# JaworWr/CUDA-ray-tracer

Measured on AMD Instinct MI355X. Metric: Mrays/sec, 20spheres.yml @1920x1080, higher is better.
Workload: dtype f64

## Files before the change

cuda-ray-tracer_amd/csrc/rt_capi.cpp:

```cpp
#include <hip/hip_runtime.h>

#include <algorithm>
#include <cmath>
#include <cstdarg>
#include <cstdio>
#include <cstdlib>
#include <cstring>
#include <memory>
#include <new>
#include <string>
#include <vector>

#include "mi355rt.h"
#include "rt_launch.h"
#include "rt_scene_dev.h"
#include "rt_scene_image.hpp"
#include "rt_frame_host.hpp"
#include "rt_set_scene.h"
#include "scene-exception.h"
#include "scene.h"
#include "camera.h"

#define RT_KERNELS(V)                                                                                                                              \
    {RT_CAT(rt_launch_trace, V), RT_CAT(rt_launch_wavefront, V),  RT_CAT(rt_launch_ray_list, V),      RT_CAT(rt_launch_gbuffer, V),   RT_CAT(rt_launch_pick, V), \
// ... 161 lines not shown
    DevMem<void> d_fb;
    DevMem<unsigned long long> d_counters;
    Event ev0, ev1;
    Event ev_done;

    hipStream_t last_stream = nullptr;
    bool rendered = false;
    bool captured = false;
    bool counted = false;
    bool zero_counters = false;
    DevMem<uint64_t> d_stamps;
    DevMem<double> d_camx, d_camy;
    size_t n_stamp_rows = 0;
    uint64_t frame = 0;
    uint32_t tag = 0;
    DevMem<uint32_t> d_order, d_tiles;
    MappedWords h_listed;
    uint32_t ord_split = 0;
    std::vector<double> cub_coefs;
    bool lean_ok = false;
    bool lean_now = true;
    uint32_t wg_slots = 1536;
    int lean_force = 0;
    bool ord_on = true;
    Staging pick;
    Staging ext;
    Staging rq;
    Scratch pth;
    DevMem<SetSceneStatus> d_ss_status;
    DevMem<unsigned char> d_ss_stage;
};

#ifdef RT_DIAGNOSTIC_BUILD
extern "C" int rt_abi_version(void) { return RT_ABI_VERSION | RT_ABI_DIAGNOSTIC; }
#else
extern "C" int rt_abi_version(void) { return RT_ABI_VERSION; }
#endif

extern "C" const char *rt_last_error(void) { return g_last_error.c_str(); }

extern "C" void rt_set_last_error(const char *message) { g_last_error = message ? message : ""; }

template <typename F>
static int scene_handle(rt_scene **out, F &&make)
{
    std::unique_ptr<rt_scene> s(new rt_scene());
// ... 207 lines not shown
    std::memset(&fa, 0, sizeof(fa));
    fa.aspect = (double) rw / rh;
    fa.tan_half_fov = std::tan(0.5 * sd->vertical_fov);
    fa.bg[0] = sd->bg_color[0];
    fa.bg[1] = sd->bg_color[1];
    fa.bg[2] = sd->bg_color[2];
    fa.bg[3] = 1.0f;
    fa.width = rw;
    fa.height = rh;
    fa.max_refl = sd->max_reflections;
    fa.rank = cfg.rank;
    fa.world = cfg.world;
    fa.band_rows = kf * cfg.band_rows;
    fa.local_rows = kf * ctx->local_rows;
    fa.tiles_x = (rw + RT_TILE - 1) / RT_TILE;
    fa.n_tiles = fa.tiles_x * ((fa.local_rows + RT_TILE - 1) / RT_TILE);
    fa.rgba8 = (ctx->ssaa == 1u && cfg.format == RT_FMT_RGBA8) ? 1u : 0u;
    fa.ord_plain = (cfg.flags & RT_FLAG_PLAIN_ORDER) ? 1u : 0u;
    ctx->ord_split = (cfg.flags & RT_FLAG_NOSPLIT) ? 0u : RT_ORD_SPLIT_CLASSES;
    if (const char *e = std::getenv("MI355RT_SPLIT_CLASSES")) ctx->ord_split = (uint32_t) std::atoi(e) & 15u;
    int cus = 0;
    if (hipDeviceGetAttribute(&cus, hipDeviceAttributeMultiprocessorCount, device) == hipSuccess && cus > 0) ctx->wg_slots = 6u * (uint32_t) cus;
    if (const char *e = std::getenv("MI355RT_LEAN")) ctx->lean_force = (e[0] == 'a') ? 1 : ((e[0] == 'n') ? -1 : 0);
}

static int create_scene(rt_ctx *ctx, const rt_scene_desc *sd, rtp::SceneImage &im)
{
    FrameArgs &fa = ctx->fa;
    im = rtp::scene_image(*sd, ctx->cfg.flags, fa);
    ctx->cub_coefs = im.cub_coefs;
    ctx->lean_ok = im.lean_ok && !std::getenv("MI355RT_NOLEAN");
    if (!(ctx->cfg.flags & RT_FLAG_SIMPLE)) {
        const size_t lds = rt_wavefront_lds_bytes_strict(fa.stage_bytes, sd->n_lights, (int) fa.has_mirror, fa.cull ? fa.n_us : 0u, 0, fa.n_cub);
        if (lds > 160u * 1024u) return fail(RT_ERR_SCENE, "rt_create: scene needs %zu bytes of LDS per workgroup (limit 160 KiB)", lds);
    }
    if (ctx->adaptive && (size_t) sd->n_objects * (sizeof(DevObject) + sizeof(UsEntry)) > 160u * 1024u)
        return fail(RT_ERR_SCENE, "rt_create: adaptive supersampling stages %zu bytes of LDS per workgroup (limit 160 KiB)",
                    (size_t) sd->n_objects * (sizeof(DevObject) + sizeof(UsEntry)));
    if (ctx->geometry && rt_gbuffer_lds_bytes_strict(&fa) > 160u * 1024u)
        return fail(RT_ERR_SCENE, "rt_create: RT_FLAG_SSAA_GEOMETRY stages %zu bytes of LDS per workgroup (limit 160 KiB)", rt_gbuffer_lds_bytes_strict(&fa));
    return RT_OK;
}

static int create_device_state(rt_ctx *ctx, const rtp::SceneImage &im)
{
    const FrameArgs &fa = ctx->fa;
// ... 44 lines not shown
    if (!ctx->geometry) return RT_OK;
    const size_t hpx = (size_t) ctx->halo_slots * width;
    std::vector<uint32_t> xy(2u * hpx);
    for (uint32_t h = 0; h < ctx->halo_slots; h++) {
        const int64_t gy = rtf::halo_global_row(h, cfg.band_rows, cfg.world, cfg.rank, ctx->local_rows);
        const uint32_t row = (uint32_t) std::min<int64_t>(std::max<int64_t>(gy, 0), (int64_t) height - 1);
        for (uint32_t x = 0; x < width; x++) {
            xy[2u * ((size_t) h * width + x)] = x;
            xy[2u * ((size_t) h * width + x) + 1u] = row;
        }
    }
    RT_TRY("hipMalloc(object plane)", ctx->d_geo_obj.alloc((px ? px : 1u) * sizeof(int32_t)));
    RT_TRY("hipMalloc(normal plane)", ctx->d_geo_nrm.alloc((px ? px : 1u) * 16u));
    if (!hpx) return RT_OK;
    RT_TRY("hipMalloc(halo records)", ctx->d_geo_halo.alloc(sizeof(rt_hit) * hpx));
    return device_table(ctx->d_geo_xy, xy.data(), sizeof(uint32_t) * 2u * hpx, "halo coordinates");
}

static int create_order_state(rt_ctx *ctx)
{
    FrameArgs &fa = ctx->fa;
    const uint32_t flags = ctx->cfg.flags;
    if (!(flags & (RT_FLAG_SIMPLE | RT_FLAG_STATIC_ORDER)) && fa.n_tiles > 0 && fa.n_tiles <= RT_ORD_MAX_TILES) {
        fa.ord_stride = (RT_ORD_HDR + 17u * fa.n_tiles + 15u) & ~15u;
        if (int rc = device_table(ctx->d_order, nullptr, sizeof(uint32_t) * (3u * (size_t) fa.ord_stride + fa.n_tiles), "order")) return rc;
        fa.order_state = ctx->d_order;
        if (hipHostMalloc((void **) &ctx->h_listed.p, 64, hipHostMallocMapped | hipHostMallocPortable) == hipSuccess) {
            ctx->h_listed[0] = 0;
            ctx->h_listed[1] = 0;
            ctx->h_listed[2] = 0xFFFFFFFFu;
            if (hipHostGetDevicePointer((void **) &fa.ord_host, ctx->h_listed, 0) != hipSuccess) {
                ctx->h_listed.reset();
                fa.ord_host = nullptr;
            }
        } else {
            ctx->h_listed.p = nullptr;
            (void) hipGetLastError();
        }
    }
    if (!(flags & RT_FLAG_SIMPLE) && fa.all_cullable && fa.n_tiles > 0) {
        if (int rc = device_table(ctx->d_tiles, nullptr, sizeof(uint32_t) * fa.n_tiles, "tile state")) return rc;
        fa.tile_state = ctx->d_tiles;
    }
    ctx->zero_counters = std::getenv("MI355RT_DEBUG_COUNTERS") != nullptr;
    if (ctx->zero_counters) {
        ctx->n_stamp_rows = (size_t) fa.n_tiles * 9 + 96;
        if (ctx->d_stamps.alloc(ctx->n_stamp_rows * 16 * sizeof(uint64_t) + 8) != hipSuccess) ctx->d_stamps.p = nullptr;
// ... 93 lines not shown
static int timer_begin(rt_ctx *ctx, hipStream_t stream, const float *ms)
{
    if (ms) RT_HIP(hipEventRecord(ctx->ev0, stream));
    return RT_OK;
}

static int timer_end(rt_ctx *ctx, hipStream_t stream, float *ms)
{
    if (!ms) return RT_OK;
    RT_HIP(hipEventRecord(ctx->ev1, stream));
    RT_HIP(hipEventSynchronize(ctx->ev1));
    RT_HIP(hipEventElapsedTime(ms, ctx->ev0, ctx->ev1));
    return RT_OK;
}

static void choose_schedule(rt_ctx *ctx, FrameArgs &fa)
{
    if (ctx->lean_ok && ctx->h_listed && ctx->lean_force == 0) {
        const uint32_t tiles = ((volatile uint32_t *) ctx->h_listed.p)[2];
        if (ctx->lean_now ? (uint64_t) tiles * 100u < (uint64_t) ctx->wg_slots * 62u : (uint64_t) tiles * 100u >= (uint64_t) ctx->wg_slots * 66u) ctx->lean_now = !ctx->lean_now;
    } else {
        ctx->lean_now = ctx->lean_force >= 0;
    }
    static const bool debug_order = std::getenv("MI355RT_DEBUG_ORDER") != nullptr;
    if (debug_order && ctx->h_listed)
        std::fprintf(stderr, "mi355rt: frame %llu: tiles with hits %u, list slots wanted %u, census %u, schedule %s\n", (unsigned long long) ctx->frame, ((volatile uint32_t *) ctx->h_listed.p)[2],
                     ((volatile uint32_t *) ctx->h_listed.p)[0], ((volatile uint32_t *) ctx->h_listed.p)[1], ctx->lean_now ? "lean" : "general");
    fa.lean = (ctx->lean_ok && ctx->lean_now && !fa.sparse) ? 1u : 0u;
}

static int rotate_launch_order(rt_ctx *ctx, FrameArgs &fa, hipStream_t stream)
{
    fa.ord_read = (uint32_t) (ctx->frame % 3u);
    fa.ord_write = (uint32_t) ((ctx->frame + 1u) % 3u);
    fa.ord_zero = (uint32_t) ((ctx->frame + 2u) % 3u);
    uint32_t cap = fa.n_tiles;
    if (ctx->h_listed) {
        const uint32_t seen = ((volatile uint32_t *) ctx->h_listed.p)[0], census = ((volatile uint32_t *) ctx->h_listed.p)[1];
        const uint64_t want = (uint64_t) seen + seen / 4u + 64u;
        if (want < cap) cap = (uint32_t) want;
        const uint64_t with_hits = (uint64_t) census * 16u;
        const uint64_t slots = ctx->wg_slots ? ctx->wg_slots : 1536u;
        const bool too_many = ctx->ord_on ? with_hits * 3u >= slots * 16u : with_hits >= slots * 4u;
        const bool too_dense = ctx->ord_on ? with_hits * 4u >= fa.n_tiles : with_hits * 5u >= fa.n_tiles;
        ctx->ord_on = !(too_many || too_dense);
    }
    fa.ord_cap = cap;
    fa.ord_on = ctx->ord_on ? 1u : 0u;
    fa.ord_split = (fa.sparse || fa.lean) ? 0u : ctx->ord_split;
    fa.ord_frame = (uint32_t) (ctx->frame % 0xFFFFFFF0ull) + 1u;
    if (fa.ord_frame == 1u && ctx->frame != 0u)
        RT_HIP(hipMemsetAsync(fa.order_state + 3u * (size_t) fa.ord_stride, 0, sizeof(uint32_t) * fa.n_tiles, stream));
    ctx->frame++;
    return RT_OK;
}

static int render_impl(rt_ctx *ctx, const double cam[16], void *dev_fb, void *stream_, float *ms, bool sparse, uint32_t sparse_cap)
{
    hipStream_t stream = (hipStream_t) stream_;
    FrameArgs &fa = ctx->fa;
    const bool ss = ctx->ssaa > 1u && !ctx->adaptive;
    const bool kernel_sparse = sparse && ctx->ssaa == 1u;
    fa.sparse = kernel_sparse ? 1u : 0u;
    fa.sparse_cap = kernel_sparse ? sparse_cap : 0u;
    choose_schedule(ctx, fa);
    rtf::frame_camera(fa, cam, ctx->cub_coefs);
    if (int rc = use_device(ctx)) return rc;
    bool capturing = false;
    if (int rc = order_begin("rt_render", ctx, stream, &capturing)) return rc;
    void *out = dev_fb ? dev_fb : ctx->d_fb.p;
    void *fb = ss ? ctx->d_ss.p : out;
// ... 721 lines not shown
```

cuda-ray-tracer_amd/csrc/rt_scene_dev.h:

```cpp
#ifndef RT_SCENE_DEV_H
#define RT_SCENE_DEV_H

#include <stddef.h>
#include <stdint.h>

enum {
    K_X3 = 0, K_Y3, K_Z3, K_X2Y, K_XY2, K_X2Z, K_XZ2, K_Y2Z, K_YZ2, K_XYZ,
    K_X2, K_Y2, K_Z2, K_XY, K_XZ, K_YZ,
    K_X, K_Y, K_Z, K_C
};

#define RT_CLS_CUBIC 1u
#define RT_CLS_SQUARE 2u
#define RT_CLS_CROSS 4u
#define RT_CLS_UNITSQ 8u

struct alignas(16) DevObject {
    double c[20];
    float albedo[3];
    float refl;
    uint32_t cls;
    uint32_t pad[3];
    double bs_center[3];
    double bs_radius;
// ... 69 lines not shown
    uint32_t has_mirror;
    uint32_t all_cullable;
    double tile_nt[9];
    double cx_a, cx_b;
    double cy_a, cy_b;
    uint32_t tile_planes_ok;
    uint32_t sparse, sparse_cap;
    uint32_t *order_state;
    uint32_t *ord_host;
    uint32_t ord_stride, ord_read, ord_write, ord_zero;
    uint32_t ord_cap;
    uint32_t ord_on;
    uint32_t ord_plain;
    uint32_t ord_frame;
    uint32_t ord_split;
    uint32_t *tile_state;
    uint32_t frame_tag;
    uint32_t n_scan;
    uint32_t lean;
    double cub_rec[4][10];
    double cub_abs[4][4];
    uint32_t lights_plain;
    uint32_t pt_mask[2];
};

#define RT_CUB_AT_MAX 4
#define RT_CUB_REC 10
static_assert(offsetof(FrameArgs, cub_abs) == offsetof(FrameArgs, cub_rec) + sizeof(double) * 4 * RT_CUB_REC, "cub_abs directly behind cub_rec");
#define RT_TILE 16
#define RT_SCAN_TILES 64
#define RT_PAINT_TILES 16
#define RT_ORD_SPLIT_CLASSES 8u
#define RT_ORD_HDR 32
#define RT_ORD_MAX_TILES 262144u

#endif
```

cuda-ray-tracer_amd/csrc/rt_wavefront.hip:

```cpp
#include <hip/hip_runtime.h>
#include <cstdlib>

#include "rt_launch.h"
#include "rt_math.hpp"
#include "rt_scene_dev.h"
#include "rt_wavefront_math.hpp"

#ifndef RT_VARIANT
#error "define RT_VARIANT=strict|fast"
#endif

namespace RT_SYM(rtw) {

using namespace rtm;

#define RT_LOAD_LIGHTK(lk, l) \
    LightK lk; \
    lk.p[0] = clight[l].p[0]; lk.p[1] = clight[l].p[1]; lk.p[2] = clight[l].p[2]; \
    lk.sdir[0] = clight[l].sdir[0]; lk.sdir[1] = clight[l].sdir[1]; lk.sdir[2] = clight[l].sdir[2]; \
    lk.u2 = clight[l].u2; lk.inv_uu = clight[l].inv_uu; lk.len_u = clight[l].len_u; lk.four_u2 = clight[l].four_u2; \
    lk.s_yz = clight[l].s_yz; lk.s_xz = clight[l].s_xz; lk.s_xy = clight[l].s_xy; \
    lk.color[0] = clight[l].color[0]; lk.color[1] = clight[l].color[1]; lk.color[2] = clight[l].color[2]; \
    lk.flags = clight[l].flags;
typedef const __attribute__((address_space(4))) LightK *ConstLights;
// ... 239 lines not shown
#pragma unroll
    for (uint32_t c = 0; c + 1 < ORD_CLASSES; c++) {
        const bool next = (k == c) && idx >= h.cnt[c];
        idx -= next ? h.cnt[c] : 0u;
        k += next ? 1u : 0u;
    }
}
__device__ __forceinline__ uint32_t ord_first(const OrdHeader &h, uint32_t k)
{
    uint32_t f = 0;
#pragma unroll
    for (uint32_t c = 0; c + 1 < ORD_CLASSES; c++) f += c < k ? h.cnt[c] : 0u;
    return f;
}
__device__ __forceinline__ uint32_t ord_rank_of_slot(uint32_t q, uint32_t n_eff, uint32_t first_block)
{
    const uint32_t off = first_block & 255u, row = (q + off) >> 8;
    if (!(row & 1u)) return q;
    const uint32_t lo = row * 256u - off;
    const uint32_t hi = (row + 1u) * 256u - off < n_eff ? (row + 1u) * 256u - off : n_eff;
    return lo + (hi - 1u - q);
}

constexpr uint32_t ST_EMPTY = 1u, ST_NONEMPTY = 2u, ST_TIMEOUT = 3u, ST_COVERED = 4u;
constexpr uint32_t ST_BITS = 3u, ST_MASK = 7u;
#ifndef RT_TILE_MAX_POLLS
#define RT_TILE_MAX_POLLS 48
#endif

__device__ __forceinline__ uint32_t tile_word_load(uint32_t *w) { return __hip_atomic_load(w, __ATOMIC_RELAXED, __HIP_MEMORY_SCOPE_AGENT); }

__device__ __forceinline__ uint32_t tile_word_wait(uint32_t *w, uint32_t tag, uint32_t v)
{
    for (int it = 0; (v >> ST_BITS) != tag; ++it) {
        if (it >= RT_TILE_MAX_POLLS) {
            uint32_t expect = v;
            if (__hip_atomic_compare_exchange_strong(w, &expect, (tag << ST_BITS) | ST_TIMEOUT, __ATOMIC_RELAXED, __ATOMIC_RELAXED, __HIP_MEMORY_SCOPE_AGENT))
                v = (tag << ST_BITS) | ST_TIMEOUT;
            else
                v = expect;
        } else {
            __builtin_amdgcn_s_sleep(16);
            v = tile_word_load(w);
        }
    }
    return v;
}

template <bool COUNT>
__device__ __forceinline__ void classify_tiles(const FrameArgs &fa, const UsEntry *us, uint32_t n_us, uint32_t *tile_state, uint32_t tag, uint32_t n_tiles,
                                               const uint32_t *ord_rd, uint32_t ord_cap, uint32_t ord_split, uint32_t wave, uint32_t lane, Cnt<COUNT> &cnt)
{
    const uint32_t i = lane & 15u, sl = lane >> 4;
    const uint32_t t = blockIdx.x * RT_SCAN_TILES + wave * 16u + i;
    const bool tv = t < n_tiles;
    uint32_t old = 0;
    if (sl == 0 && tv) old = tile_word_load(tile_state + t);
    double kx = 0.0, ky = 0.0, kz = 0.0, r = 0.0, inv = 0.0;
    if (sl < n_us) {
        const UsEntry *e = us + sl;
        kx = e->kx; ky = e->ky; kz = e->kz; r = e->r; inv = e->inv_r;
    }
    const uint32_t tc = tv ? t : n_tiles - 1u;
    const uint32_t tile_x = tc % fa.tiles_x, tile_y = tc / fa.tiles_x;
    const uint32_t x0 = tile_x * RT_TILE, y0l = tile_y * RT_TILE;
    const uint32_t x1 = x0 + RT_TILE - 1 < fa.width ? x0 + RT_TILE - 1 : fa.width - 1;
    const uint32_t y1l = y0l + RT_TILE - 1 < fa.local_rows ? y0l + RT_TILE - 1 : fa.local_rows - 1;
    const double gy0 = (double) global_row(fa, y0l), gy1 = (double) global_row(fa, y1l);
    const TilePlanes P = tile_planes(fa, fa.cx_a * ((double) x0 - 0.5) + fa.cx_b, fa.cx_a * ((double) x1 + 0.5) + fa.cx_b,
                                     fa.cy_a * (gy0 - 0.5) + fa.cy_b, fa.cy_a * (gy1 + 0.5) + fa.cy_b);
    const D3 org{fa.origin[0], fa.origin[1], fa.origin[2]};
    bool rel = sl < n_us && sphere_in_pyramid(kx, ky, kz, r, inv, org, P);
    for (uint32_t base = 4; base < n_us; base += 4) {
        const uint32_t j = base + sl;
        if (j < n_us) {
            const UsEntry *e = us + j;
            rel = rel || sphere_in_pyramid(e->kx, e->ky, e->kz, e->r, e->inv_r, org, P);
        }
    }
    if (!fa.tile_planes_ok) rel = true;
    unsigned long long m = __ballot(rel);
    m |= m >> 32;
    m |= m >> 16;
    const bool nonempty = (m >> i) & 1ull;
    if (sl == 0 && tv && (old >> ST_BITS) != tag) {
        uint32_t st = nonempty ? ST_NONEMPTY : ST_EMPTY;
        if (nonempty && ord_rd) {
            const OrdHeader oh = ord_header(ord_rd, ord_split);
            const uint32_t n_eff = ord_positions(oh) < ord_cap ? ord_positions(oh) : ord_cap;
            const uint32_t w = ord_rd[RT_ORD_HDR + t];
            const uint32_t cls = w & 31u, pos = w >> 5;
            if (cls >= 1u && cls <= ORD_CLASSES && pos < n_tiles) {
                const uint32_t k = cls - 1u;
                uint32_t count = 0;
#pragma unroll
                for (uint32_t c = 0; c < ORD_CLASSES; c++) count = c == k ? oh.cnt[c] : count;
                if (pos < count && ord_last_position(oh, ord_first(oh, k) + pos) < n_eff && ord_rd[RT_ORD_HDR + (1u + k) * n_tiles + pos] == t) st = ST_COVERED;
            }
        }
        uint32_t expect = old;
        __hip_atomic_compare_exchange_strong(tile_state + t, &expect, (tag << ST_BITS) | st, __ATOMIC_RELAXED, __ATOMIC_RELAXED,
                                             __HIP_MEMORY_SCOPE_AGENT);
    }
    if (lane == 0) {
        const uint32_t first = blockIdx.x * RT_SCAN_TILES + wave * 16u;
        const uint32_t nt = first >= n_tiles ? 0u : (n_tiles - first < 16u ? n_tiles - first : 16u);
        cnt.cull(C_TILE, (unsigned long long) nt * n_us);
    }
}

// ... 575 lines not shown
                if (hit) {
                    res.x = (acc.x < 1.0f) ? acc.x : 1.0f;
                    res.y = (acc.y < 1.0f) ? acc.y : 1.0f;
                    res.z = (acc.z < 1.0f) ? acc.z : 1.0f;
                }
                if (listing_) b_ticks = __builtin_amdgcn_s_memtime() - b_t0;
                RT_STAMP(6);
            }
    }

template <bool COUNT, bool HAS_GQ, bool HAS_CUBIC, bool HAS_MIRROR, bool LEAN = false>
__global__ __launch_bounds__(256, (wf_occupancy<COUNT, HAS_GQ, HAS_CUBIC, HAS_MIRROR, LEAN>())) void wavefront_tile_kernel(
    const unsigned char *hot_us,
    const uint32_t *hot_ord_rd,
    uint32_t hot_n_us, uint32_t hot_ord_cap, uint32_t hot_n_tiles,
    uint32_t hot_flags,
    uint32_t *hot_tile_state,
    uint32_t hot_frame_tag, uint32_t hot_n_scan,
    const ColdArgs cold_never_named)
{
    const uint32_t tid = threadIdx.x, wave = (uint32_t) __builtin_amdgcn_readfirstlane((int) (threadIdx.x >> 6)), lane = tid & 63;
    constexpr bool ALL_SPHERES_POSSIBLE = !HAS_GQ && !HAS_CUBIC;
    const uint32_t ord_slots = (hot_flags & 2u) ? hot_ord_cap : 0u;
    uint32_t slot = blockIdx.x;
    uint32_t tstate = ST_TIMEOUT;
    uint32_t role = 0, paint_block = 0;
    if (ALL_SPHERES_POSSIBLE && hot_tile_state) {
        if (blockIdx.x < hot_n_scan) {
            role = 1;
        } else {
            slot -= hot_n_scan;
            if (slot >= ord_slots) {
                const uint32_t q = slot - ord_slots;
                if (hot_flags & 4u) {
                    const uint32_t grp = q / (RT_PAINT_TILES + 1u), pos = q - grp * (RT_PAINT_TILES + 1u);
                    if (pos == 0u) {
                        role = 2;
                        paint_block = grp;
                    }
                    slot = ord_slots + grp * RT_PAINT_TILES + (pos - 1u);
                    if (role == 0 && slot - ord_slots >= hot_n_tiles) return;
                }
                if (role == 0) {
                    uint32_t *w = hot_tile_state + (slot - ord_slots);
                    uint32_t v = 0;
                    if (lane == 0) v = tile_word_wait(w, hot_frame_tag, tile_word_load(w));
// ... 44 lines not shown
    unsigned long long *sblk = reinterpret_cast<unsigned long long *>(smem + L.shadow);
    Ball *sball = reinterpret_cast<Ball *>(smem + L.ball);
    BoxH *sbox = reinterpret_cast<BoxH *>(smem + L.box);
    CullRec *screc = reinterpret_cast<CullRec *>(smem + L.crec);
    uint32_t *s_wcount = reinterpret_cast<uint32_t *>(smem + L.misc);
    uint32_t *s_live = s_wcount + 4;
    uint32_t *s_sparse = s_wcount + 8;
    uint32_t *s_zero = s_wcount + 10;
    uint32_t *s_decode = s_wcount + 12;
    uint32_t *s_half = s_wcount + 11;
    uint32_t *s_cost = s_wcount + 9;
    uint32_t *s_done = s_wcount + 15;

    RT_STAMP_DECL
    const uint32_t stamp_row_base_ = 0u;
    (void) stamp_row_base_;
    bool staged = false;
    RT_STAMP(0);

    Cnt<COUNT> cnt;
    const F3 bg{fa.bg[0], fa.bg[1], fa.bg[2]};

    if (ALL_SPHERES_POSSIBLE && role == 1) {
        classify_tiles<COUNT>(fa, reinterpret_cast<const UsEntry *>(hot_us), hot_n_us, hot_tile_state, hot_frame_tag, hot_n_tiles,
                              (hot_flags & 2u) ? hot_ord_rd : nullptr, hot_ord_cap, ((hot_flags >> 4) & 15u) | ((hot_flags >> 20) << 4), wave, lane, cnt);
        RT_STAMP(11);
        RT_STAMP_FLUSH(counters, lane);
        cnt.flush(counters);
        return;
    }
    if (ALL_SPHERES_POSSIBLE && role == 2) {
        paint_tiles(fa, hot_tile_state, hot_frame_tag, hot_n_tiles, fb, bg, paint_block, wave, lane);
        RT_STAMP(11);
        RT_STAMP_FLUSH(counters, lane);
        return;
    }
#ifdef RT_WF_DEBUG_EXITS
    if ((hot_flags & 0x100u) && slot >= ord_slots) return;
#endif

    double pkx = 0.0, pky = 0.0, pkz = 0.0, pr = 0.0, pinv = 0.0;
    if (ALL_SPHERES_POSSIBLE && (hot_flags & 1u) && wave == 0 && lane < hot_n_us) {
        const UsEntry *pe = reinterpret_cast<const UsEntry *>(hot_us) + lane;
        pkx = pe->kx; pky = pe->ky; pkz = pe->kz; pr = pe->r; pinv = pe->inv_r;
    }
    uint32_t *ord_wr = nullptr;
    uint32_t tile = slot;
    bool listed = false;
    uint32_t half = 0;
    bool listing = false;
    uint32_t cost_scale = 0;
    bool covered = false;
    if (fa.order_state && !fa.ord_on) {
        ord_wr = fa.order_state + (size_t) fa.ord_write * fa.ord_stride;
        if (slot == 0 && tid == 0) {
            const uint32_t *ord_rd = fa.order_state + (size_t) fa.ord_read * fa.ord_stride;
            uint32_t *z = fa.order_state + (size_t) fa.ord_zero * fa.ord_stride;
            for (uint32_t k = 0; k < RT_ORD_HDR; k += 4) *reinterpret_cast<uint4 *>(z + k) = make_uint4(0, 0, 0, 0);
            if (fa.ord_host) { fa.ord_host[0] = 0; fa.ord_host[1] = ord_rd[16]; fa.ord_host[2] = ord_rd[16] * 16u; }
        }
    }
    if (hot_flags & 2u) {
        ord_wr = fa.order_state + (size_t) fa.ord_write * fa.ord_stride;
        asm volatile("" ::"s"(fa.cam[0]), "s"(fa.cam[2]), "s"(fa.cam[5]), "s"(fa.cam[6]), "s"(fa.cam[8]), "s"(fa.cam[10]), "s"(fa.origin[0]),
                     "s"(fa.origin[2]), "s"(fa.aspect), "s"(fa.tan_half_fov), "s"(fa.width), "s"(fa.local_rows), "s"(fa.tiles_x), "s"(fa.n_us),
                     "s"(fa.off_us), "s"(fa.band_rows), "s"(fa.all_cullable), "s"(gscene));
        if (wave == 0) {
            typedef const __attribute__((address_space(4))) uint32_t *ConstWords;
            ConstWords ord_rd = (ConstWords) hot_ord_rd;
            const OrdHeader oh = ord_header(ord_rd, ((hot_flags >> 4) & 15u) | ((hot_flags >> 20) << 4));
            const uint32_t idx_tile = slot >= ord_slots ? slot - ord_slots : 0u;
            const uint32_t w = ord_rd[RT_ORD_HDR + idx_tile];
            const uint32_t n_eff = ord_positions(oh) < hot_ord_cap ? ord_positions(oh) : hot_ord_cap;
            if (slot == 0 && lane == 0) {
                uint32_t *z = fa.order_state + (size_t) fa.ord_zero * fa.ord_stride;
                for (uint32_t k = 0; k < RT_ORD_HDR; k += 4) *reinterpret_cast<uint4 *>(z + k) = make_uint4(0, 0, 0, 0);
                if (fa.ord_host) { fa.ord_host[0] = oh.n_listed + oh.n_candidates; fa.ord_host[1] = oh.census; fa.ord_host[2] = oh.n_listed; }
            }
            uint32_t d_half = 0;
            uint32_t d_tile = slot, d_flags = oh.census * 64u < hot_n_tiles ? 4u : 0u;
            if (slot < ord_slots) {
                if (slot >= n_eff) {
                    d_flags |= 8u;
                } else {
                    const uint32_t p = (hot_flags & 8u) ? slot : ord_rank_of_slot(slot, n_eff, blockIdx.x - slot);
                    const uint32_t rank = p < 2u * oh.n_heavy ? p >> 1 : p - oh.n_heavy;
                    d_half = p < 2u * oh.n_heavy ? 1u + (p & 1u) : 0u;
                    uint32_t k, idx;
                    ord_locate(oh, rank, k, idx);
                    d_tile = ord_rd[RT_ORD_HDR + (1u + k) * hot_n_tiles + idx];
                    const uint32_t back = ord_rd[RT_ORD_HDR + (d_tile < hot_n_tiles ? d_tile : 0u)];
                    d_flags |= (d_tile >= hot_n_tiles || back != ((idx << 5) | (k + 1u)) || ord_last_position(oh, rank) >= n_eff) ? 8u : 1u;
                }
            } else {
                d_tile = idx_tile;
                const uint32_t cls = w & 31u, pos = w >> 5;
                if ((tstate == ST_TIMEOUT || (COUNT && tstate == ST_EMPTY)) && cls >= 1u && cls <= ORD_CLASSES && pos < hot_n_tiles) {
                    const uint32_t k = cls - 1u;
                    uint32_t count = 0;
#pragma unroll
                    for (uint32_t c = 0; c < ORD_CLASSES; c++) count = c == k ? oh.cnt[c] : count;
                    if (pos < count && ord_last_position(oh, ord_first(oh, k) + pos) < n_eff && ord_rd[RT_ORD_HDR + (1u + k) * hot_n_tiles + pos] == d_tile) d_flags |= 2u;
                }
            }
            if (lane == 0) { s_decode[0] = d_tile; s_decode[1] = d_flags; s_decode[2] = oh.cost_max; s_half[0] = d_half; }
        }
        if (LEAN) RT_STAMP(3);
        lds_barrier();
        if (LEAN) RT_STAMP(4);
        tile = (uint32_t) __builtin_amdgcn_readfirstlane((int) s_decode[0]);
        const uint32_t d_flags = (uint32_t) __builtin_amdgcn_readfirstlane((int) s_decode[1]);
        cost_scale = (uint32_t) __builtin_amdgcn_readfirstlane((int) s_decode[2]);
        if (d_flags & 8u) return;
        listed = (d_flags & 1u) != 0u;
        covered = (d_flags & 2u) != 0u;
        listing = (d_flags & 4u) != 0u;
        half = (uint32_t) __builtin_amdgcn_readfirstlane((int) s_half[0]);
    }
#ifdef RT_WF_DEBUG_EXITS
    if ((hot_flags & 0x200u) && !listed) {
        asm volatile("" ::"s"(tile), "s"((uint32_t) covered), "s"(tstate));
        return;
    }
#endif
    {
        asm volatile("" ::"s"(fa.width), "s"(fa.local_rows), "s"(fa.tiles_x), "s"(fa.band_rows), "s"(fa.rank), "s"(fa.world), "s"(fa.all_cullable),
                     "s"(fa.tile_planes_ok));
        const uint32_t tile_x = tile % fa.tiles_x, tile_y = tile / fa.tiles_x;
        const uint32_t x = tile_x * RT_TILE + tile_px(tid), lr = tile_y * RT_TILE + tile_py(tid);
        const bool inside = x < fa.width && lr < fa.local_rows && (half == 0u || (tid >> 7) + 1u == half);
        const uint32_t xc = x < fa.width ? x : fa.width - 1, lrc = lr < fa.local_rows ? lr : fa.local_rows - 1;
        const uint32_t y = global_row(fa, lrc);

        if (ALL_SPHERES_POSSIBLE && tstate == ST_EMPTY) {
            if (COUNT && !covered && inside) {
                cnt.add(0);
                cnt.add(3, fa.n_obj);
            }
            RT_STAMP_FLUSH(counters, lane);
            cnt.flush(counters);
// ... 54 lines not shown
            lds_barrier();
        }

        if (covered) return;
        const uint4 *stage_scene = reinterpret_cast<const uint4 *>(gscene + fa.off_us);
        const uint4 *stage_light = reinterpret_cast<const uint4 *>(glight);
        const uint32_t n16 = fa.stage_bytes / 16, tot16 = n16;
        uint4 pre0 = make_uint4(0, 0, 0, 0), pre1 = make_uint4(0, 0, 0, 0);
        if (tid < tot16) pre0 = tid < n16 ? stage_scene[tid] : stage_light[tid - n16];
        if (tid + WG < tot16) pre1 = tid + WG < n16 ? stage_scene[tid + WG] : stage_light[tid + WG - n16];
        F3 res = bg;
        D3 o{fa.origin[0], fa.origin[1], fa.origin[2]};
#if RT_WF_CAMTAB
        D3 dir = primary_dir_tab(fa, camx[xc], camy[y]);
#else
        D3 dir = primary_dir(fa, (int) xc, (int) y);
#endif
        if (ALL_SPHERES_POSSIBLE && fa.all_cullable) {
            uint4 *dst = reinterpret_cast<uint4 *>(smem + L.scene);
            if (tid < tot16) dst[tid] = pre0;
            if (tid + WG < tot16) dst[tid + WG] = pre1;
            for (uint32_t i = tid + 2 * WG; i < tot16; i += WG) dst[i] = i < n16 ? stage_scene[i] : stage_light[i - n16];
            staged = true;
            if (LEAN && tid == 0) { s_done[0] = 0u; s_cost[0] = 0u; s_zero[0] = 0u; if (!(hot_flags & 2u)) s_half[0] = 0u; }
            if (LEAN) RT_STAMP(7);
            lds_barrier();
            if (LEAN) RT_STAMP(8);
        }
        bool live = inside;
        uint32_t ord_cls = 0, ord_pos = 0;
        if constexpr (LEAN) {
            unsigned long long hm = 0ull, b_ticks = 0ull;
            LeanLds M;
            M.hp = hp; M.hp_stride = WG; M.sball = sball; M.sbox = sbox; M.screc = screc; M.smem = smem; M.crec_off = L.crec; M.n_crec = L.n_crec;
            lean_block<COUNT>(fa, S, gobj, M, glight, cnt, tile, o, dir, live, listing, lane, tid, wave, res, hm, b_ticks RT_STAMP_PASS);
            if (ord_wr && lane == 0) {
                if (hm != 0ull) __hip_atomic_fetch_add(&s_cost[0], (uint32_t) (b_ticks >> 6) + 1u, __ATOMIC_RELAXED, __HIP_MEMORY_SCOPE_WORKGROUP);
                const uint32_t before = __hip_atomic_fetch_add(&s_done[0], 1u, __ATOMIC_ACQ_REL, __HIP_MEMORY_SCOPE_WORKGROUP);
                if (before == 3u) {
                    const uint32_t cost4 = __hip_atomic_load(&s_cost[0], __ATOMIC_RELAXED, __HIP_MEMORY_SCOPE_WORKGROUP);
                    const uint32_t cost = (cost4 + 3u) >> 2;
                    if (cost != 0u) {
                        if (((tile * 0x9E3779B1u) >> 28) == 0u) atomicAdd(&ord_wr[16], 1u);
                        if (listing) {
                            const uint32_t q = cost_scale ? (uint32_t) (((unsigned long long) cost * ORD_CLASSES) / ((unsigned long long) cost_scale + 1ull)) : 0u;
                            ord_cls = ORD_CLASSES - (q < ORD_CLASSES - 1u ? q : ORD_CLASSES - 1u);
                            ord_pos = atomicAdd(&ord_wr[ord_cls - 1u], 1u);
                            if (cost > cost_scale - cost_scale / 4u || ((tile * 0x9E3779B1u) >> 28) == 0u) atomicMax(&ord_wr[17], cost);
                        }
                    }
                }
            }
        } else {
        bool first = true;
        if (HAS_CUBIC && fa.n_cub != 0u) {
            double *prim = reinterpret_cast<double *>(smem + L.cubprim);
            if (lane < (RT_CUB_REC + 4) * RT_CUB_AT_MAX) prim[lane] = (&fa.cub_rec[0][0])[lane];
            __builtin_amdgcn_fence(__ATOMIC_RELEASE, "wavefront", "local");
            __builtin_amdgcn_fence(__ATOMIC_ACQUIRE, "wavefront", "local");
        }
        if (fa.sparse && tid == 0) s_sparse[0] = 0xFFFFFFFFu;
        if (!(hot_flags & 2u) && tid == 0) s_half[0] = 0u;
        if (tid == 0) s_zero[0] = 0u;
        float cur_ratio = 1.0f;
        uint32_t n_refl = 0;
        if (inside) cnt.add(0);
        cnt.primary_traced();

        RT_STAMP(1);
        for (;;) {
// ... 292 lines not shown
                    reinterpret_cast<float4 *>(msg + off_tiles)[mpix] = make_float4(res.x, res.y, res.z, 1.0f);
                }
                if (tid == 0) msg[4u + mslot] = tile;
            } else if (mslot != 0xFFFFFFFFu && tid == 0) {
                msg[1] = 1u;
            }
        } else if (sx_ < fe.width && sy_ < fe.local_rows && (s_half[0] == 0u || (tid_ >> 7) + 1u == s_half[0])) {
            const size_t pix = (size_t) sy_ * fe.width + sx_;
            if (fe.rgba8) {
                uchar4 px;
                px.x = (unsigned char) (int) (res.x * 255.0f + 0.5f);
                px.y = (unsigned char) (int) (res.y * 255.0f + 0.5f);
                px.z = (unsigned char) (int) (res.z * 255.0f + 0.5f);
                px.w = 255;
                reinterpret_cast<uchar4 *>(fb)[pix] = px;
            } else {
                reinterpret_cast<float4 *>(fb)[pix] = make_float4(res.x, res.y, res.z, 1.0f);
            }
        }
        if (ord_cls && ord_pos < fe.n_tiles) {
            ord_wr[RT_ORD_HDR + ord_cls * fe.n_tiles + ord_pos] = tile;
            ord_wr[RT_ORD_HDR + tile] = (ord_pos << 5) | ord_cls;
        }
        RT_STAMP(10);
    }

    RT_STAMP_FLUSH(counters, lane);
    cnt.flush(counters);
}


}

extern "C" size_t RT_SYM(rt_wavefront_lds_bytes)(uint32_t stage_bytes, uint32_t n_lights, int has_mirror, uint32_t n_cull_spheres, int lean, uint32_t n_cub)
{
    return RT_SYM(rtw)::LdsLayout(stage_bytes, n_lights, has_mirror != 0, n_cull_spheres, lean != 0, n_cub).total;
}

extern "C" hipError_t RT_SYM(rt_launch_wavefront)(const FrameArgs *fa, const DevObject *gobj, const DevLight *glight,
                                                   void *fb, unsigned long long *counters, int count,
                                                   const double *camx, const double *camy, hipStream_t stream)
{
    using namespace RT_SYM(rtw);
    if (fa->n_tiles == 0) return hipSuccess;
    const uint32_t n_scan = fa->tile_state ? fa->n_scan : 0u;
    const uint32_t n_paint = (n_scan && !fa->sparse) ? (fa->n_tiles + RT_PAINT_TILES - 1u) / RT_PAINT_TILES : 0u;
    const uint32_t n_index = n_paint ? n_paint * (RT_PAINT_TILES + 1u) : fa->n_tiles;
    const dim3 grid(n_scan + ((fa->order_state && fa->ord_on) ? fa->ord_cap : 0u) + n_index), block(WG);
    const unsigned char *gs = reinterpret_cast<const unsigned char *>(gobj);
    int sel = (count ? 8 : 0) | (fa->has_mirror ? 4 : 0) | (fa->n_gq ? 2 : 0) | (fa->n_cub ? 1 : 0);
    const bool lean = fa->lean && (sel & 7) == 0 && fa->all_cullable && fa->n_us == fa->n_obj && !fa->sparse;
    if (lean) sel = count ? 17 : 16;
    const size_t lds = LdsLayout(fa->stage_bytes, fa->n_lights, fa->has_mirror != 0, fa->cull ? fa->n_us : 0u, lean, fa->n_cub).total;
    const bool ordering = fa->order_state && fa->ord_on;
    const unsigned char *hot_us = gs + fa->off_us;
    const uint32_t *hot_ord_rd = ordering ? fa->order_state + (size_t) fa->ord_read * fa->ord_stride : nullptr;
    uint32_t hot_flags = (fa->all_cullable ? 1u : 0u) | (ordering ? 2u : 0u) | (n_paint ? 4u : 0u) | (fa->ord_plain ? 8u : 0u) |
                         ((fa->ord_split & 15u) << 4);
#ifdef RT_WF_DEBUG_EXITS
    if (const char *dbg = getenv("MI355RT_DEBUG_EXIT")) hot_flags |= (uint32_t) atoi(dbg) << 8;
#endif
    if (fa->ord_split && ordering) {
        struct SlotsKey { int dev, sel; size_t lds; uint32_t slots; };
        static thread_local SlotsKey memo[4] = {{-1, 0, 0, 0}, {-1, 0, 0, 0}, {-1, 0, 0, 0}, {-1, 0, 0, 0}};
        static thread_local unsigned memo_next = 0;
        int dev = 0;
        (void) hipGetDevice(&dev);
        uint32_t slots = 0;
        bool found = false;
        for (const SlotsKey &k : memo)
            if (k.dev == dev && k.sel == sel && k.lds == lds) { slots = k.slots; found = true; }
        if (!found) {
            int per_cu = 0, cus = 0;
#define RT_OCC(C, M, G, Q) (void) hipOccupancyMaxActiveBlocksPerMultiprocessor(&per_cu, wavefront_tile_kernel<C, G, Q, M>, WG, lds)
            switch (sel) {
            case 0: RT_OCC(false, false, false, false); break;
            case 1: RT_OCC(false, false, false, true); break;
            case 2: RT_OCC(false, false, true, false); break;
            case 3: RT_OCC(false, false, true, true); break;
            case 4: RT_OCC(false, true, false, false); break;
            case 5: RT_OCC(false, true, false, true); break;
// ... 38 lines not shown
```

Measured before the change: 205,900.

## Add sharded flat tile-order list for lean schedule

```diff
diff --git a/cuda-ray-tracer_amd/csrc/rt_capi.cpp b/cuda-ray-tracer_amd/csrc/rt_capi.cpp
--- a/cuda-ray-tracer_amd/csrc/rt_capi.cpp
+++ b/cuda-ray-tracer_amd/csrc/rt_capi.cpp
@@ -207,6 +207,8 @@
     bool lean_now = true;
     uint32_t wg_slots = 1536;
     int lean_force = 0;
+    bool debug_order = false;
+    bool lean_flat = true;
     bool ord_on = true;
     Staging pick;
     Staging ext;
@@ -460,6 +462,8 @@
     int cus = 0;
     if (hipDeviceGetAttribute(&cus, hipDeviceAttributeMultiprocessorCount, device) == hipSuccess && cus > 0) ctx->wg_slots = 6u * (uint32_t) cus;
     if (const char *e = std::getenv("MI355RT_LEAN")) ctx->lean_force = (e[0] == 'a') ? 1 : ((e[0] == 'n') ? -1 : 0);
+    ctx->debug_order = std::getenv("MI355RT_DEBUG_ORDER") != nullptr;
+    if (const char *e = std::getenv("MI355RT_LEAN_ORDER")) ctx->lean_flat = e[0] != 'c';
 }
 
 static int create_scene(rt_ctx *ctx, const rt_scene_desc *sd, rtp::SceneImage &im)
@@ -550,7 +554,7 @@
     FrameArgs &fa = ctx->fa;
     const uint32_t flags = ctx->cfg.flags;
     if (!(flags & (RT_FLAG_SIMPLE | RT_FLAG_STATIC_ORDER)) && fa.n_tiles > 0 && fa.n_tiles <= RT_ORD_MAX_TILES) {
-        fa.ord_stride = (RT_ORD_HDR + 17u * fa.n_tiles + 15u) & ~15u;
+        fa.ord_stride = RT_ORD_STRIDE(fa.n_tiles);
         if (int rc = device_table(ctx->d_order, nullptr, sizeof(uint32_t) * (3u * (size_t) fa.ord_stride + fa.n_tiles), "order")) return rc;
         fa.order_state = ctx->d_order;
         if (hipHostMalloc((void **) &ctx->h_listed.p, 64, hipHostMallocMapped | hipHostMallocPortable) == hipSuccess) {
@@ -690,8 +694,7 @@
     } else {
         ctx->lean_now = ctx->lean_force >= 0;
     }
-    static const bool debug_order = std::getenv("MI355RT_DEBUG_ORDER") != nullptr;
-    if (debug_order && ctx->h_listed)
+    if (ctx->debug_order && ctx->h_listed)
         std::fprintf(stderr, "mi355rt: frame %llu: tiles with hits %u, list slots wanted %u, census %u, schedule %s\n", (unsigned long long) ctx->frame, ((volatile uint32_t *) ctx->h_listed.p)[2],
                      ((volatile uint32_t *) ctx->h_listed.p)[0], ((volatile uint32_t *) ctx->h_listed.p)[1], ctx->lean_now ? "lean" : "general");
     fa.lean = (ctx->lean_ok && ctx->lean_now && !fa.sparse) ? 1u : 0u;
@@ -715,6 +718,7 @@
     }
     fa.ord_cap = cap;
     fa.ord_on = ctx->ord_on ? 1u : 0u;
+    fa.ord_flat = (fa.lean && ctx->lean_flat) ? 1u : 0u;
     fa.ord_split = (fa.sparse || fa.lean) ? 0u : ctx->ord_split;
     fa.ord_frame = (uint32_t) (ctx->frame % 0xFFFFFFF0ull) + 1u;
     if (fa.ord_frame == 1u && ctx->frame != 0u)
diff --git a/cuda-ray-tracer_amd/csrc/rt_scene_dev.h b/cuda-ray-tracer_amd/csrc/rt_scene_dev.h
--- a/cuda-ray-tracer_amd/csrc/rt_scene_dev.h
+++ b/cuda-ray-tracer_amd/csrc/rt_scene_dev.h
@@ -115,6 +115,7 @@
     double cub_abs[4][4];
     uint32_t lights_plain;
     uint32_t pt_mask[2];
+    uint32_t ord_flat;
 };
 
 #define RT_CUB_AT_MAX 4
@@ -126,5 +127,13 @@
 #define RT_ORD_SPLIT_CLASSES 8u
 #define RT_ORD_HDR 32
 #define RT_ORD_MAX_TILES 262144u
+#define RT_ORD_FLAT_SHARDS 16u
+#define RT_ORD_FLAT_LINE 32u
+#define RT_ORD_FLAT_SHARD(t) (((t) ^ ((t) >> 4) ^ ((t) >> 8)) & 15u)
+#define RT_ORD_FLAT_CNT(n) ((RT_ORD_HDR + 17u * (n) + 31u) & ~31u)
+#define RT_ORD_FLAT_LIST(n) (RT_ORD_FLAT_CNT(n) + RT_ORD_FLAT_SHARDS * RT_ORD_FLAT_LINE)
+#define RT_ORD_FLAT_CAP(n) (((n) + 15u) & ~15u)
+#define RT_ORD_FLAT_WORD(n) (RT_ORD_FLAT_LIST(n) + RT_ORD_FLAT_CAP(n))
+#define RT_ORD_STRIDE(n) ((RT_ORD_FLAT_WORD(n) + (n) + 31u) & ~31u)
 
 #endif
diff --git a/cuda-ray-tracer_amd/csrc/rt_wavefront.hip b/cuda-ray-tracer_amd/csrc/rt_wavefront.hip
--- a/cuda-ray-tracer_amd/csrc/rt_wavefront.hip
+++ b/cuda-ray-tracer_amd/csrc/rt_wavefront.hip
@@ -285,6 +285,30 @@
     return lo + (hi - 1u - q);
 }
 
+struct FlatSlot { uint32_t tile; bool valid; };
+template <typename Words>
+__device__ __forceinline__ FlatSlot ord_flat_slot(Words rd, uint32_t q, uint32_t n_tiles)
+{
+    const uint32_t e = rd[RT_ORD_FLAT_LIST(n_tiles) + q], count = rd[RT_ORD_FLAT_CNT(n_tiles) + (q & 15u) * RT_ORD_FLAT_LINE];
+    const bool in = (q >> 4) < count && e < n_tiles;
+    const uint32_t back = rd[RT_ORD_FLAT_WORD(n_tiles) + (in ? e : 0u)];
+    return FlatSlot{e, in && back == q + 1u};
+}
+template <typename Words>
+__device__ __forceinline__ bool ord_flat_covered(Words rd, uint32_t t, uint32_t n_tiles, uint32_t list_slots)
+{
+    const uint32_t w = rd[RT_ORD_FLAT_WORD(n_tiles) + t], q = w - 1u;
+    if (w == 0u || q >= list_slots || q >= RT_ORD_FLAT_CAP(n_tiles)) return false;
+    return (q >> 4) < rd[RT_ORD_FLAT_CNT(n_tiles) + (q & 15u) * RT_ORD_FLAT_LINE] && rd[RT_ORD_FLAT_LIST(n_tiles) + q] == t;
+}
+template <bool FLAT>
+__device__ __forceinline__ void ord_clear(uint32_t *z, uint32_t n_tiles)
+{
+    for (uint32_t k = 0; k < RT_ORD_HDR; k += 4) *reinterpret_cast<uint4 *>(z + k) = make_uint4(0, 0, 0, 0);
+    if constexpr (FLAT)
+        for (uint32_t s = 0; s < RT_ORD_FLAT_SHARDS; s++) z[RT_ORD_FLAT_CNT(n_tiles) + s * RT_ORD_FLAT_LINE] = 0u;
+}
+
 constexpr uint32_t ST_EMPTY = 1u, ST_NONEMPTY = 2u, ST_TIMEOUT = 3u, ST_COVERED = 4u;
 constexpr uint32_t ST_BITS = 3u, ST_MASK = 7u;
 #ifndef RT_TILE_MAX_POLLS
@@ -310,9 +334,9 @@
     return v;
 }
 
-template <bool COUNT>
+template <bool COUNT, bool FLAT_POSSIBLE>
 __device__ __forceinline__ void classify_tiles(const FrameArgs &fa, const UsEntry *us, uint32_t n_us, uint32_t *tile_state, uint32_t tag, uint32_t n_tiles,
-                                               const uint32_t *ord_rd, uint32_t ord_cap, uint32_t ord_split, uint32_t wave, uint32_t lane, Cnt<COUNT> &cnt)
+                                               const uint32_t *ord_rd, uint32_t ord_cap, uint32_t ord_split, bool flat, uint32_t wave, uint32_t lane, Cnt<COUNT> &cnt)
 {
     const uint32_t i = lane & 15u, sl = lane >> 4;
     const uint32_t t = blockIdx.x * RT_SCAN_TILES + wave * 16u + i;
@@ -348,7 +372,9 @@
     const bool nonempty = (m >> i) & 1ull;
     if (sl == 0 && tv && (old >> ST_BITS) != tag) {
         uint32_t st = nonempty ? ST_NONEMPTY : ST_EMPTY;
-        if (nonempty && ord_rd) {
+        if (FLAT_POSSIBLE && flat) {
+            if (nonempty && ord_flat_covered(ord_rd, t, n_tiles, ord_cap)) st = ST_COVERED;
+        } else if (nonempty && ord_rd) {
             const OrdHeader oh = ord_header(ord_rd, ord_split);
             const uint32_t n_eff = ord_positions(oh) < ord_cap ? ord_positions(oh) : ord_cap;
             const uint32_t w = ord_rd[RT_ORD_HDR + t];
@@ -970,6 +996,9 @@
     const uint32_t tid = threadIdx.x, wave = (uint32_t) __builtin_amdgcn_readfirstlane((int) (threadIdx.x >> 6)), lane = tid & 63;
     constexpr bool ALL_SPHERES_POSSIBLE = !HAS_GQ && !HAS_CUBIC;
     const uint32_t ord_slots = (hot_flags & 2u) ? hot_ord_cap : 0u;
+    constexpr bool FLAT_POSSIBLE = LEAN && !COUNT;
+    constexpr bool LEAN_SCENES = !HAS_GQ && !HAS_CUBIC && !HAS_MIRROR;
+    const bool flat = FLAT_POSSIBLE && (hot_flags & 0x800u) != 0u;
     uint32_t slot = blockIdx.x;
     uint32_t tstate = ST_TIMEOUT;
     uint32_t role = 0, paint_block = 0;
@@ -1060,8 +1089,8 @@
     const F3 bg{fa.bg[0], fa.bg[1], fa.bg[2]};
 
     if (ALL_SPHERES_POSSIBLE && role == 1) {
-        classify_tiles<COUNT>(fa, reinterpret_cast<const UsEntry *>(hot_us), hot_n_us, hot_tile_state, hot_frame_tag, hot_n_tiles,
-                              (hot_flags & 2u) ? hot_ord_rd : nullptr, hot_ord_cap, ((hot_flags >> 4) & 15u) | ((hot_flags >> 20) << 4), wave, lane, cnt);
+        classify_tiles<COUNT, FLAT_POSSIBLE>(fa, reinterpret_cast<const UsEntry *>(hot_us), hot_n_us, hot_tile_state, hot_frame_tag, hot_n_tiles,
+                                             (hot_flags & 2u) ? hot_ord_rd : nullptr, hot_ord_cap, ((hot_flags >> 4) & 15u) | ((hot_flags >> 20) << 4), flat, wave, lane, cnt);
         RT_STAMP(11);
         RT_STAMP_FLUSH(counters, lane);
         cnt.flush(counters);
@@ -1093,8 +1122,7 @@
         ord_wr = fa.order_state + (size_t) fa.ord_write * fa.ord_stride;
         if (slot == 0 && tid == 0) {
             const uint32_t *ord_rd = fa.order_state + (size_t) fa.ord_read * fa.ord_stride;
-            uint32_t *z = fa.order_state + (size_t) fa.ord_zero * fa.ord_stride;
-            for (uint32_t k = 0; k < RT_ORD_HDR; k += 4) *reinterpret_cast<uint4 *>(z + k) = make_uint4(0, 0, 0, 0);
+            ord_clear<LEAN_SCENES>(fa.order_state + (size_t) fa.ord_zero * fa.ord_stride, hot_n_tiles);
             if (fa.ord_host) { fa.ord_host[0] = 0; fa.ord_host[1] = ord_rd[16]; fa.ord_host[2] = ord_rd[16] * 16u; }
         }
     }
@@ -1103,16 +1131,40 @@
         asm volatile("" ::"s"(fa.cam[0]), "s"(fa.cam[2]), "s"(fa.cam[5]), "s"(fa.cam[6]), "s"(fa.cam[8]), "s"(fa.cam[10]), "s"(fa.origin[0]),
                      "s"(fa.origin[2]), "s"(fa.aspect), "s"(fa.tan_half_fov), "s"(fa.width), "s"(fa.local_rows), "s"(fa.tiles_x), "s"(fa.n_us),
                      "s"(fa.off_us), "s"(fa.band_rows), "s"(fa.all_cullable), "s"(gscene));
+        typedef const __attribute__((address_space(4))) uint32_t *ConstWords;
+        ConstWords ord_rd = (ConstWords) hot_ord_rd;
+        if (flat) {
+            const uint32_t census = ord_rd[16];
+            cost_scale = ord_rd[17];
+            listing = census * 64u < hot_n_tiles;
+            if (slot < ord_slots) {
+                const FlatSlot fs = ord_flat_slot(ord_rd, slot, hot_n_tiles);
+                if (slot == 0 && wave == 0) {
+                    uint32_t n_listed = 0;
+#pragma unroll
+                    for (uint32_t k = 0; k < ORD_CLASSES; k++) n_listed += ord_rd[k];
+                    if (lane == 0) {
+                        ord_clear<LEAN_SCENES>(fa.order_state + (size_t) fa.ord_zero * fa.ord_stride, hot_n_tiles);
+                        if (fa.ord_host) { fa.ord_host[0] = n_listed; fa.ord_host[1] = census; fa.ord_host[2] = n_listed; }
+                    }
+                }
+                if (LEAN) { RT_STAMP(3); RT_STAMP(4); }
+                if (!fs.valid) return;
+                tile = fs.tile;
+                listed = true;
+            } else {
+                tile = slot - ord_slots;
+                if (tstate == ST_TIMEOUT) covered = ord_flat_covered(ord_rd, tile, hot_n_tiles, ord_slots);
+                if (LEAN) { RT_STAMP(3); RT_STAMP(4); }
+            }
+        } else {
         if (wave == 0) {
-            typedef const __attribute__((address_space(4))) uint32_t *ConstWords;
-            ConstWords ord_rd = (ConstWords) hot_ord_rd;
             const OrdHeader oh = ord_header(ord_rd, ((hot_flags >> 4) & 15u) | ((hot_flags >> 20) << 4));
             const uint32_t idx_tile = slot >= ord_slots ? slot - ord_slots : 0u;
             const uint32_t w = ord_rd[RT_ORD_HDR + idx_tile];
             const uint32_t n_eff = ord_positions(oh) < hot_ord_cap ? ord_positions(oh) : hot_ord_cap;
             if (slot == 0 && lane == 0) {
-                uint32_t *z = fa.order_state + (size_t) fa.ord_zero * fa.ord_stride;
-                for (uint32_t k = 0; k < RT_ORD_HDR; k += 4) *reinterpret_cast<uint4 *>(z + k) = make_uint4(0, 0, 0, 0);
+                ord_clear<LEAN_SCENES>(fa.order_state + (size_t) fa.ord_zero * fa.ord_stride, hot_n_tiles);
                 if (fa.ord_host) { fa.ord_host[0] = oh.n_listed + oh.n_candidates; fa.ord_host[1] = oh.census; fa.ord_host[2] = oh.n_listed; }
             }
             uint32_t d_half = 0;
@@ -1154,6 +1206,7 @@
         covered = (d_flags & 2u) != 0u;
         listing = (d_flags & 4u) != 0u;
         half = (uint32_t) __builtin_amdgcn_readfirstlane((int) s_half[0]);
+        }
     }
 #ifdef RT_WF_DEBUG_EXITS
     if ((hot_flags & 0x200u) && !listed) {
@@ -1254,13 +1307,14 @@
             if (tid + WG < tot16) dst[tid + WG] = pre1;
             for (uint32_t i = tid + 2 * WG; i < tot16; i += WG) dst[i] = i < n16 ? stage_scene[i] : stage_light[i - n16];
             staged = true;
-            if (LEAN && tid == 0) { s_done[0] = 0u; s_cost[0] = 0u; s_zero[0] = 0u; if (!(hot_flags & 2u)) s_half[0] = 0u; }
+            if (LEAN && tid == 0) { s_done[0] = 0u; s_cost[0] = 0u; s_zero[0] = 0u; if (!(hot_flags & 2u) || flat) s_half[0] = 0u; }
             if (LEAN) RT_STAMP(7);
             lds_barrier();
             if (LEAN) RT_STAMP(8);
         }
         bool live = inside;
         uint32_t ord_cls = 0, ord_pos = 0;
+        uint32_t ord_fq = 0xFFFFFFFFu;
         if constexpr (LEAN) {
             unsigned long long hm = 0ull, b_ticks = 0ull;
             LeanLds M;
@@ -1278,6 +1332,8 @@
                             const uint32_t q = cost_scale ? (uint32_t) (((unsigned long long) cost * ORD_CLASSES) / ((unsigned long long) cost_scale + 1ull)) : 0u;
                             ord_cls = ORD_CLASSES - (q < ORD_CLASSES - 1u ? q : ORD_CLASSES - 1u);
                             ord_pos = atomicAdd(&ord_wr[ord_cls - 1u], 1u);
+                            const uint32_t shard = RT_ORD_FLAT_SHARD(tile);
+                            ord_fq = atomicAdd(&ord_wr[RT_ORD_FLAT_CNT(hot_n_tiles) + shard * RT_ORD_FLAT_LINE], 1u) * RT_ORD_FLAT_SHARDS + shard;
                             if (cost > cost_scale - cost_scale / 4u || ((tile * 0x9E3779B1u) >> 28) == 0u) atomicMax(&ord_wr[17], cost);
                         }
                     }
@@ -1616,6 +1672,10 @@
             ord_wr[RT_ORD_HDR + ord_cls * fe.n_tiles + ord_pos] = tile;
             ord_wr[RT_ORD_HDR + tile] = (ord_pos << 5) | ord_cls;
         }
+        if (LEAN && ord_fq < RT_ORD_FLAT_CAP(fe.n_tiles)) {
+            ord_wr[RT_ORD_FLAT_LIST(fe.n_tiles) + ord_fq] = tile;
+            ord_wr[RT_ORD_FLAT_WORD(fe.n_tiles) + tile] = ord_fq + 1u;
+        }
         RT_STAMP(10);
     }
 
@@ -1650,7 +1710,8 @@
     const unsigned char *hot_us = gs + fa->off_us;
     const uint32_t *hot_ord_rd = ordering ? fa->order_state + (size_t) fa->ord_read * fa->ord_stride : nullptr;
     uint32_t hot_flags = (fa->all_cullable ? 1u : 0u) | (ordering ? 2u : 0u) | (n_paint ? 4u : 0u) | (fa->ord_plain ? 8u : 0u) |
-                         ((fa->ord_split & 15u) << 4);
+                         ((fa->ord_split & 15u) << 4) |
+                         ((ordering && lean && !count && fa->ord_flat) ? 0x800u : 0u);
 #ifdef RT_WF_DEBUG_EXITS
     if (const char *dbg = getenv("MI355RT_DEBUG_EXIT")) hot_flags |= (uint32_t) atoi(dbg) << 8;
 #endif
```

New measurement: 174,100. -15.4%, worse.
